# mmetcalf14/qml-cutensornet

Measured on AMD Instinct MI355X. Metric: Gram kernel entries/sec @ 60 qubits x 6 layers, higher is better.
Workload: dtype f64 (complex128)

## Files before the change

qml-cutensornet_amd/csrc/qk_fused.h:

```cpp
#pragma once
#include "qk_device.h"
#include "qk_plan.h"

#define QKF_PRIO_LO() __builtin_amdgcn_s_setprio(0)
#define QKF_PRIO_HI() __builtin_amdgcn_s_setprio(2)
typedef double v2d __attribute__((ext_vector_type(2)));
typedef __attribute__((address_space(3))) v2d lds_v2d;
static constexpr int QKF_XSTEP = 4 * TILE;
static constexpr int QKF_XBLOCK = TILE * TILE;


#ifndef QKF_LDS3M
#define QKF_LDS3M 0
#endif
#ifndef QKF_P2_PROBE
#define QKF_P2_PROBE 0
#endif
#ifndef QKF_ABL
#define QKF_ABL 0
#endif
#define QKF_STEP_BARRIER()                            \
  do {                                                \
    if (QKF_ABL & 4) asm volatile("s_waitcnt lgkmcnt(0)" ::: "memory"); \
    else qk_lds_barrier();                            \
// ... 219 lines not shown
  }
}

#ifdef QKF_EDGE_PAIRS_V
#define QKF_EDGE_PAIRS(WPS) (QKF_EDGE_PAIRS_V != 0)
#else
#define QKF_EDGE_PAIRS(WPS) false
#endif
#ifdef QKF_EDGE_SETS_V
#define QKF_EDGE_SETS(WPS) (QKF_EDGE_SETS_V)
#else
#define QKF_EDGE_SETS(WPS) ((WPS) <= 3 ? 2 : 1)
#endif
__device__ __forceinline__ v2d qkf_lde(const v2d* __restrict__ base, const unsigned boff, const int col = 0) {
  return reinterpret_cast<const v2d*>(reinterpret_cast<const char*>(base) + (size_t)boff)[col];
}
template <bool HAS1, bool MORE>
__device__ __forceinline__ void qkf_edge_group(v4d (&acc)[6], v2d (&fy)[4], v2d (&fz)[4], v2d (&fx)[4], const v2d* const* const by, const v2d* const* const bx, const unsigned boy,
                                               const unsigned box) {
#pragma unroll
  for (int i = 0; i < 4; ++i) {
    const double sb = QKF_DIF(fx[i].x, fx[i].y);
    acc[0] = __builtin_amdgcn_mfma_f64_16x16x4f64(fy[i].x, fx[i].x, acc[0], 0, 0, 0);
    acc[1] = __builtin_amdgcn_mfma_f64_16x16x4f64(fy[i].y, fx[i].y, acc[1], 0, 0, 0);
    acc[2] = __builtin_amdgcn_mfma_f64_16x16x4f64(QKF_SUM(fy[i].x, fy[i].y), sb, acc[2], 0, 0, 0);
    if (HAS1) {
      acc[3] = __builtin_amdgcn_mfma_f64_16x16x4f64(fz[i].x, fx[i].x, acc[3], 0, 0, 0);
      acc[4] = __builtin_amdgcn_mfma_f64_16x16x4f64(fz[i].y, fx[i].y, acc[4], 0, 0, 0);
      acc[5] = __builtin_amdgcn_mfma_f64_16x16x4f64(QKF_SUM(fz[i].x, fz[i].y), sb, acc[5], 0, 0, 0);
    }
    if (MORE) {
      fy[i] = qkf_lde(by[i], boy);
      if (HAS1) fz[i] = qkf_lde(by[i], boy, TILE);
      fx[i] = qkf_lde(bx[i], box);
    }
    __builtin_amdgcn_sched_barrier(0);
  }
}
template <bool HAS1, int SETS>
__device__ __forceinline__ void qkf_edge_unit(QkfTile& t0, QkfTile& t1, const v2d* __restrict__ Ay, const unsigned oy, const int ldy, const v2d* __restrict__ Ax, const unsigned ox, const int ldx,
                                              const int ng) {
  static_assert(SETS == 1 || SETS == 2, "one or two groups of k-steps in flight");
  v4d acc[6];
#pragma unroll
  for (int e = 0; e < 6; ++e) acc[e] = (v4d){0, 0, 0, 0};
  v2d fy[SETS][4], fz[SETS][4], fx[SETS][4];
  const v2d *by[4 * SETS], *bx[4 * SETS];
#pragma unroll
  for (int i = 0; i < 4 * SETS; ++i) by[i] = Ay + 4 * i * ldy, bx[i] = Ax + 4 * i * ldx;
  unsigned boy = oy * 16u, box = ox * 16u;
  const unsigned sy = (unsigned)(SETS * TILE * ldy) * 16u, sx = (unsigned)(SETS * TILE * ldx) * 16u;
  const bool two = SETS == 2 && ng > 1;
#pragma unroll
  for (int s = 0; s < SETS; ++s) {
    if (s == 0 || two) {
#pragma unroll
      for (int i = 0; i < 4; ++i) {
        fy[s][i] = qkf_lde(by[4 * s + i], boy);
        if (HAS1) fz[s][i] = qkf_lde(by[4 * s + i], boy, TILE);
        fx[s][i] = qkf_lde(bx[4 * s + i], box);
      }
    }
  }
  QKF_PRIO_LO();
#pragma unroll 1
  for (int g = SETS; g < ng; g += SETS) {
    boy += sy, box += sx;
#pragma unroll
    for (int s = 0; s < SETS; ++s) qkf_edge_group<HAS1, true>(acc, fy[s], fz[s], fx[s], by + 4 * s, bx + 4 * s, boy, box);
  }
  qkf_edge_group<HAS1, false>(acc, fy[0], fz[0], fx[0], by, bx, boy, box);
  if constexpr (SETS == 2) {
    if (two) qkf_edge_group<HAS1, false>(acc, fy[1], fz[1], fx[1], by + 4, bx + 4, boy, box);
  }
  QKF_PRIO_HI();
  t0.re = acc[0] + acc[1], t0.im = acc[2] - acc[0] + acc[1];
  if (HAS1) t1.re = acc[3] + acc[4], t1.im = acc[5] - acc[3] + acc[4];
}
__device__ __forceinline__ long long qkf_uniform(const long long v) {
  const unsigned lo = __builtin_amdgcn_readfirstlane((unsigned)v);
  const unsigned hi = __builtin_amdgcn_readfirstlane((unsigned)((unsigned long long)v >> 32));
  return (long long)(((unsigned long long)hi << 32) | lo);
}

template <int NW, bool PAIRS>
__device__ __forceinline__ QkEdgeUnit qkf_edge_unit_of(const int u, const int mt, const int nt, const int inv) {
  if constexpr (PAIRS) return qk_edge_unit(u, mt, nt, NW, inv);
  const int tb = (u * inv) >> 20;
  return QkEdgeUnit{u - tb * mt, tb, false, true};
}
template <int NW, bool PAIRS, int SETS>
__device__ __forceinline__ void qkf_edge_prefix(const SweepArgs& g, const int xi, const int yj, const int a, const int b, lds_v2d* const xl, v2d* const xg, const bool to_global, const int wave,
                                                const int q, const int j) {
  const v2d* const Lx = reinterpret_cast<const v2d*>(g.xedge) + qkf_uniform(g.xedge_offs[2 * (long long)xi]);
  const v2d* const Ly = reinterpret_cast<const v2d*>(g.yedge) + qkf_uniform(g.yedge_offs[2 * (long long)yj]);
  const int mt = a / TILE, nt = b / TILE, ng = (1 << g.edge_k) >> 4, inv = qk_recip20(mt), units = PAIRS ? qk_edge_units(mt, nt, NW) : mt * nt;
  for (int u = wave; u < units; u += NW) {
    const QkEdgeUnit un = qkf_edge_unit_of<NW, PAIRS>(u, mt, nt, inv);
    if (!un.mine) continue;
    QkfTile T0, T1;
    const unsigned oy = (unsigned)(q * b + un.tb0 * TILE + j), ox = (unsigned)(q * a + un.ta * TILE + j);
    if (un.has1) qkf_edge_unit<true, 1>(T0, T1, Ly, oy, b, Lx, ox, a, ng);
    else qkf_edge_unit<false, SETS>(T0, T1, Ly, oy, b, Lx, ox, a, ng);
    const int at = un.ta * (b * TILE) + (un.tb0 * TILE + q) * TILE + j;
    if (to_global) {
#pragma unroll
      for (int r = 0; r < 4; ++r) xg[at + r * QKF_XSTEP] = (v2d){T0.re[r], T0.im[r]};
      if (un.has1) {
#pragma unroll
        for (int r = 0; r < 4; ++r) xg[at + QKF_XBLOCK + r * QKF_XSTEP] = (v2d){T1.re[r], T1.im[r]};
      }
    } else {
#pragma unroll
      for (int r = 0; r < 4; ++r) xl[at + r * QKF_XSTEP] = (v2d){T0.re[r], T0.im[r]};
      if (un.has1) {
#pragma unroll
        for (int r = 0; r < 4; ++r) xl[at + QKF_XBLOCK + r * QKF_XSTEP] = (v2d){T1.re[r], T1.im[r]};
      }
    }
  }
}

template <int NW, bool PAIRS, int SETS>
__device__ __forceinline__ void qkf_edge_suffix(const SweepArgs& g, const int xi, const int yj, const int a, const int b, const lds_v2d* const xl, const v2d* const xg, const bool from_global,
                                                __attribute__((address_space(3))) double* zacc, const int wave, const int q, const int j) {
  const v2d* const Rx = reinterpret_cast<const v2d*>(g.xedge) + qkf_uniform(g.xedge_offs[2 * (long long)xi + 1]);
  const v2d* const Ry = reinterpret_cast<const v2d*>(g.yedge) + qkf_uniform(g.yedge_offs[2 * (long long)yj + 1]);
  const int mt = a / TILE, nt = b / TILE, ng = (1 << g.edge_k) >> 4, inv = qk_recip20(mt), units = PAIRS ? qk_edge_units(mt, nt, NW) : mt * nt;
  double zr = 0, zi = 0;
  for (int u = wave; u < units; u += NW) {
    const QkEdgeUnit un = qkf_edge_unit_of<NW, PAIRS>(u, mt, nt, inv);
    if (!un.mine) continue;
    QkfTile T0, T1;
    const unsigned oy = (unsigned)(q * b + un.tb0 * TILE + j), ox = (unsigned)(q * a + un.ta * TILE + j);
    if (un.has1) qkf_edge_unit<true, 1>(T0, T1, Ry, oy, b, Rx, ox, a, ng);
    else qkf_edge_unit<false, SETS>(T0, T1, Ry, oy, b, Rx, ox, a, ng);
    const int at = un.ta * (b * TILE) + (un.tb0 * TILE + q) * TILE + j;
#pragma unroll
    for (int r = 0; r < 4; ++r) {
      const v2d x = from_global ? xg[at + r * QKF_XSTEP] : (v2d)xl[at + r * QKF_XSTEP];
      zr += x.x * T0.re[r] - x.y * T0.im[r], zi += x.x * T0.im[r] + x.y * T0.re[r];
    }
    if (un.has1) {
#pragma unroll
      for (int r = 0; r < 4; ++r) {
        const v2d x = from_global ? xg[at + QKF_XBLOCK + r * QKF_XSTEP] : (v2d)xl[at + QKF_XBLOCK + r * QKF_XSTEP];
        zr += x.x * T1.re[r] - x.y * T1.im[r], zi += x.x * T1.im[r] + x.y * T1.re[r];
      }
    }
  }
#pragma unroll
  for (int o = 32; o > 0; o >>= 1) zr += __shfl_xor(zr, o), zi += __shfl_xor(zi, o);
  if ((q | j) == 0) zacc[2 * wave] = zr, zacc[2 * wave + 1] = zi;
}

struct QkfSite {
  int a, a2, b, b2, at, nks, mt, nt, nn, W, inv, inv2, pd, ps, next;
  bool small;
  const v2d *Ak, *Bk;
};
typedef int v4i __attribute__((ext_vector_type(4)));
typedef __attribute__((address_space(3))) v4i lds_v4i;

template <int XCAP, int NT, bool ITEM_RECIPS = false, typename OneRound>
__device__ __forceinline__ void qkf_step_table(const SweepArgs& g, const int xi, const int yj, lds_v4i* const rec, long long* const m_off, const int tid, const OneRound one_round) {
  const int ns = g.n_sites, n1 = ns + 1;
  const int32_t* const xd = g.xdims + (long long)xi * n1;
  const int32_t* const yd = g.ydims + (long long)yj * n1;
  const int32_t* const xt = g.xtrue + (long long)xi * n1;
  const int32_t* const yt = g.ytrue + (long long)yj * n1;
  const v2d* const xdata = reinterpret_cast<const v2d*>(g.xdata);
  const v2d* const ydata = reinterpret_cast<const v2d*>(g.ydata);
  auto is_small = [&](const int a, const int a2, const int b, const int b2, const int pd) __attribute__((always_inline)) {
    return a * b <= XCAP && a2 * b2 <= XCAP && (one_round(pd * (a / TILE), b2 / TILE) || a * b + a2 * b2 <= XCAP);
  };
  auto put = [&](const int e, const int a, const int a2, const int b, const int b2, const int ps, const int next, const bool small, const v2d* const A, const v2d* const B)
                 __attribute__((always_inline)) {
    const int mt = a / TILE, nt = b2 / TILE;
    const int W = small ? nt : max(1, min(nt, XCAP / (TILE * a2)));
    rec[3 * e] = (v4i){a, a2, b, b2};
    rec[3 * e + 1] = (v4i){xt[e], (yt[e] + 3) >> 2, W, small ? 1 : 0};
    rec[3 * e + 2] = (v4i){qk_recip20(mt), ps, next, ITEM_RECIPS ? qk_unit_recips(nt, W, false) : 0};
    m_off[2 * e] = (long long)(((const char*)A - (const char*)xdata) / 16);
    m_off[2 * e + 1] = (long long)(((const char*)B - (const char*)ydata) / 16);
  };
  auto plain = [&](const int e, const int next) __attribute__((always_inline)) {
    const int a = xd[e], a2 = xd[e + 1], b = yd[e], b2 = yd[e + 1];
    put(e, a, a2, b, b2, 1, next, is_small(a, a2, b, b2, 2), xdata + (g.xoffs[(long long)xi * ns + e] >> 1), ydata + (g.yoffs[(long long)yj * ns + e] >> 1));
  };
  if (g.merge_steps == 0) {
    for (int e = tid; e < ns; e += NT) plain(e, e + 1);
    return;
  }
  const int ek = g.edge_k, k_hi = ns - ek;
  for (int t = tid; 2 * t < k_hi - ek; t += NT) {
    const int e = ek + 2 * t;
    if (e + 1 >= k_hi) {
      plain(e, e + 1);
      continue;
    }
    const int a = xd[e], am = xd[e + 1], a2 = xd[e + 2], b = yd[e], bm = yd[e + 1], b2 = yd[e + 2];
    const bool sm = is_small(a, a2, b, b2, 4);
    const long long work_m = 4ll * a * b2 * (b + a2), work_p = 2ll * a * bm * (b + am) + 2ll * am * b2 * (bm + a2);
    const bool merged = (sm || (!is_small(a, am, b, bm, 2) && !is_small(am, a2, bm, b2, 2))) && work_m <= work_p;
    plain(e + 1, e + 2);
    if (merged)
      put(e, a, a2, b, b2, 2, e + 2, sm, reinterpret_cast<const v2d*>(g.xmg) + (g.xmg_offs[(long long)xi * g.merge_steps + t] >> 1),
          reinterpret_cast<const v2d*>(g.ymg) + (g.ymg_offs[(long long)yj * g.merge_steps + t] >> 1));
    else plain(e, e + 1);
  }
}

#ifdef QKF_PROF
#define QKF_PROF_DECL() \
  unsigned long long pf[8] = {0, 0, 0, 0, 0, 0, 0, 0}, pt = __builtin_amdgcn_s_memtime(); \
  const unsigned long long pt0 = pt
#define QKF_STAMP(i)                                              \
  do {                                                            \
    const unsigned long long now_ = __builtin_amdgcn_s_memtime(); \
    pf[i] += now_ - pt;                                           \
    pt = now_;                                                    \
  } while (0)
#define QKF_PROF_FLUSH()                                             \
  do {                                                               \
    if (lane == 0) {                                                 \
      pf[7] = __builtin_amdgcn_s_memtime() - pt0;                    \
      for (int i_ = 0; i_ < 8; ++i_) atomicAdd(g.prof + i_, pf[i_]); \
    }                                                                \
  } while (0)
#else
#define QKF_PROF_DECL()
#define QKF_STAMP(i)
#define QKF_PROF_FLUSH()
#endif

#define QKF_PULLER(NT) ((NT) - 64)
__device__ __forceinline__ void qkf_pull_next(const SweepArgs& g, const int xcc, int& gang_round, long long* const word) {
  const long long pp = qk_pull(g, xcc);
  qk_gang_sync(g, xcc, pp >= 0, gang_round);
  *word = pp;
}

template <int NW, int S, int XCAP, int WPS, bool DET = false>
__global__ __launch_bounds__(64 * NW, WPS) void qk_sweep_fused_kernel(const SweepArgs g) {
  constexpr int NT = 64 * NW;
  extern __shared__ __attribute__((aligned(16))) double lds_raw[];
  lds_v2d* const XL = (lds_v2d*)lds_raw;
  long long* const slot = reinterpret_cast<long long*>(lds_raw + 2 * XCAP);
  const v2d* const xdata = reinterpret_cast<const v2d*>(g.xdata);
  const v2d* const ydata = reinterpret_cast<const v2d*>(g.ydata);
  v2d* const G0 = reinterpret_cast<v2d*>(g.scratch) + (long long)blockIdx.x * 2 * g.x_plane;
  const int tid = threadIdx.x, lane = tid & 63;
  const int wave = __builtin_amdgcn_readfirstlane(tid >> 6);
  const int j = lane & 15, q = lane >> 4;
  const int ns = g.n_sites;
  __attribute__((address_space(3))) double* const zacc = (__attribute__((address_space(3))) double*)(slot + 2);
  lds_v4i* const rec = (lds_v4i*)(slot + 2 + 32);
  long long* const m_off = reinterpret_cast<long long*>(slot + 2 + 32) + 6 * (long long)ns;
  lds_int* const tbroken = (lds_int*)(m_off + 2 * (long long)ns);
  lds_int* const turn0 = tbroken + 2;
  auto rfl = [&](const int v) __attribute__((always_inline)) { return __builtin_amdgcn_readfirstlane(v); };
  auto ldl = [&](const long long* p_) __attribute__((always_inline)) {
    const long long v = *p_;
    const unsigned lo = __builtin_amdgcn_readfirstlane((unsigned)v);
    const unsigned hi = __builtin_amdgcn_readfirstlane((unsigned)((unsigned long long)v >> 32));
    return (long long)(((unsigned long long)hi << 32) | lo);
  };
  auto site = [&](const int k) __attribute__((always_inline)) {
    const v4i r0 = rec[3 * k], r1 = rec[3 * k + 1], r2 = rec[3 * k + 2];
    QkfSite s;
    s.a = rfl(r0.x), s.a2 = rfl(r0.y), s.b = rfl(r0.z), s.b2 = rfl(r0.w);
    s.at = rfl(r1.x), s.nks = rfl(r1.y), s.W = rfl(r1.z), s.small = rfl(r1.w) != 0;
    s.inv = rfl(r2.x), s.inv2 = rfl(r2.w);
    s.ps = rfl(r2.y), s.pd = 1 << s.ps, s.next = rfl(r2.z);
    s.mt = s.a / TILE, s.nt = s.b2 / TILE, s.nn = s.a2 / TILE;
    s.Ak = xdata + ldl(m_off + 2 * k);
    s.Bk = ydata + ldl(m_off + 2 * k + 1);
    return s;
  };
  auto item_of = [&](const QkfSite& s, const int w, const int it) __attribute__((always_inline)) {
    return DET ? qk_unit_decode_ordered(it, s.ps, s.mt, s.inv) : qk_unit_decode(it, s.mt, w, s.inv, qk_unit_recip_of(s.inv2, w == s.W));
  };
  auto b_stream = [&](const QkfSite& s, const int s0, const int w, const int it) __attribute__((always_inline)) {
    const QkUnit un = item_of(s, w, it);
    return QkfStream{s.Bk + un.p * s.b2, (unsigned)((q * s.pd) * s.b2 + (s0 + un.tc) * TILE + j), 4 * s.pd * s.b2, min(4, s.nks)};
  };
  auto a_stream = [&](const QkfSite& s, const int w, const int it) __attribute__((always_inline)) {
    const QkUnit un = item_of(s, w, it);
    return QkfStream{s.Ak + un.p * s.a2, (unsigned)(((un.ta * TILE + q) * s.pd) * s.a2 + j), 4 * s.pd * s.a2, min(4, (s.at - un.ta * TILE + 3) >> 2)};
  };
  QKF_PROF_DECL();
  const int xcc = qk_xcc_id();
  int gang_round = 0;
  if (tid == 0) qk_tail_start(g);
  for (;;) {
    if (tid == 0) {
      const long long pp_ = qk_pull(g, xcc);
      qk_gang_sync(g, xcc, pp_ >= 0, gang_round);
      *slot = pp_;
    }
    __syncthreads();
    const long long p = *slot;
    __syncthreads();
    if (p < 0) break;
    const int xi = g.pairs[2 * p], yj = g.pairs[2 * p + 1];
    qkf_step_table<XCAP, NT, true>(g, xi, yj, rec, m_off, tid, [](const int pmt, const int nt) { return pmt * nt <= NW * S; });
// ... 226 lines not shown
#endif
      p1 = __builtin_amdgcn_mfma_f64_16x16x4f64(s0[i], fr[i].x, p1, 0, 0, 0);
      p2 = __builtin_amdgcn_mfma_f64_16x16x4f64(t0.re[i], sp, p2, 0, 0, 0);
      p3 = __builtin_amdgcn_mfma_f64_16x16x4f64(t0.im[i], sm, p3, 0, 0, 0);
      if (HAS1) {
        r1 = __builtin_amdgcn_mfma_f64_16x16x4f64(s1[i], fr[i].x, r1, 0, 0, 0);
        r2 = __builtin_amdgcn_mfma_f64_16x16x4f64(t1.re[i], sp, r2, 0, 0, 0);
        r3 = __builtin_amdgcn_mfma_f64_16x16x4f64(t1.im[i], sm, r3, 0, 0, 0);
      }
    }
    if (!(QKF_ABL & 2)) fr[i] = qkf_ldg_a(i == 0 ? b0 : i == 1 ? b1 : i == 2 ? b2 : b3, off);
    __builtin_amdgcn_sched_barrier(0);
  }
  QKF_PRIO_HI();
#if QKF_LDS3M
#pragma unroll
  for (int r = 0; r < 4; ++r) {
    __hip_atomic_fetch_add(d + r * rs, p1[r], __ATOMIC_RELAXED, __HIP_MEMORY_SCOPE_WORKGROUP);
    __hip_atomic_fetch_add(d + r * rs + 1, p1[r], __ATOMIC_RELAXED, __HIP_MEMORY_SCOPE_WORKGROUP);
    __hip_atomic_fetch_add(d + r * rs, p3[r], __ATOMIC_RELAXED, __HIP_MEMORY_SCOPE_WORKGROUP);
    __hip_atomic_fetch_add(d + r * rs + 1, p2[r], __ATOMIC_RELAXED, __HIP_MEMORY_SCOPE_WORKGROUP);
  }
  if (HAS1) {
#pragma unroll
    for (int r = 0; r < 4; ++r) {
      __hip_atomic_fetch_add(d1 + r * rs, r1[r], __ATOMIC_RELAXED, __HIP_MEMORY_SCOPE_WORKGROUP);
      __hip_atomic_fetch_add(d1 + r * rs + 1, r1[r], __ATOMIC_RELAXED, __HIP_MEMORY_SCOPE_WORKGROUP);
      __hip_atomic_fetch_add(d1 + r * rs, r3[r], __ATOMIC_RELAXED, __HIP_MEMORY_SCOPE_WORKGROUP);
      __hip_atomic_fetch_add(d1 + r * rs + 1, r2[r], __ATOMIC_RELAXED, __HIP_MEMORY_SCOPE_WORKGROUP);
    }
  }
#elif QKF_P2_PROBE
  {
    const v4d re = p1 - p3, im = p1 - p2, re1 = r1 - r3, im1 = r1 - r2;
    lds_double* const e = d - (threadIdx.x & 63);
    lds_double* const e1 = e + 2 * QKF_XBLOCK;
#pragma unroll
    for (int r = 0; r < 4; ++r) {
      if (QKF_P2_PROBE == 1) {
        __hip_atomic_fetch_add(e + r * 64, re[r], __ATOMIC_RELAXED, __HIP_MEMORY_SCOPE_WORKGROUP);
        __hip_atomic_fetch_add(e + r * 64 + 256, im[r], __ATOMIC_RELAXED, __HIP_MEMORY_SCOPE_WORKGROUP);
        if (HAS1) {
          __hip_atomic_fetch_add(e1 + r * 64, re1[r], __ATOMIC_RELAXED, __HIP_MEMORY_SCOPE_WORKGROUP);
          __hip_atomic_fetch_add(e1 + r * 64 + 256, im1[r], __ATOMIC_RELAXED, __HIP_MEMORY_SCOPE_WORKGROUP);
        }
      } else if (QKF_P2_PROBE == 2) {
        *(lds_v2d*)(d + r * rs) = (v2d){re[r], im[r]};
        if (HAS1) *(lds_v2d*)(d1 + r * rs) = (v2d){re1[r], im1[r]};
      } else if (QKF_P2_PROBE == 3) {
        asm volatile("" ::"v"(re[r]), "v"(im[r]), "v"(re1[r]), "v"(im1[r]));
      } else {
        asm volatile("" ::"v"(p1[r]), "v"(p2[r]), "v"(p3[r]), "v"(r1[r]), "v"(r2[r]), "v"(r3[r]));
      }
    }
  }
#else
  {
    const v4d re = p1 - p3, im = p1 - p2;
#pragma unroll
    for (int r = 0; r < 4; ++r) {
      __hip_atomic_fetch_add(d + r * rs, re[r], __ATOMIC_RELAXED, __HIP_MEMORY_SCOPE_WORKGROUP);
      __hip_atomic_fetch_add(d + r * rs + 1, im[r], __ATOMIC_RELAXED, __HIP_MEMORY_SCOPE_WORKGROUP);
    }
  }
  if (HAS1) {
    const v4d re = r1 - r3, im = r1 - r2;
#pragma unroll
    for (int r = 0; r < 4; ++r) {
      __hip_atomic_fetch_add(d1 + r * rs, re[r], __ATOMIC_RELAXED, __HIP_MEMORY_SCOPE_WORKGROUP);
      __hip_atomic_fetch_add(d1 + r * rs + 1, im[r], __ATOMIC_RELAXED, __HIP_MEMORY_SCOPE_WORKGROUP);
    }
  }
#endif
}
template <bool FULL, bool HAS1, bool DET>
__device__ __forceinline__ void qkf_p2_dual_turn(const QkfTile& t0, const QkfTile& t1, v2d (&fr)[4], v2d (&fs)[4], QkfStream cur, const int ps, const int nn, const int kmax, lds_v2d* xo, const int q,
                                            const int j, const QkfStream nxt, const bool nxt_p1, const unsigned n1, const QkfTurn turn = QkfTurn{nullptr, 0, nullptr, nullptr}) {
  __attribute__((address_space(3))) double* d = (__attribute__((address_space(3))) double*)(xo + q * TILE + j);
#pragma unroll 1
  for (int tn = 0; tn < nn; ++tn) {
    v4d p1 = {0, 0, 0, 0}, p2 = {0, 0, 0, 0}, p3 = {0, 0, 0, 0}, r1 = {0, 0, 0, 0}, r2 = {0, 0, 0, 0}, r3 = {0, 0, 0, 0};
    const bool fin = tn + 1 == nn;
    const v2d* const rb = fin ? nxt.base : cur.base;
    const int rs = fin ? nxt.step : cur.step;
    cur.off = fin ? nxt.off : cur.off + TILE;
    QKF_PRIO_LO();
#pragma unroll
    for (int i = 0; i < 4; ++i) {
      if (FULL || i < kmax) {
        qkf_kstep<true>(p1, p2, p3, t0.re[i], t0.im[i], fr[i].x, fr[i].y);
        if (HAS1) qkf_kstep<true>(r1, r2, r3, t1.re[i], t1.im[i], fr[i].x, fr[i].y);
      }
      fr[i] = qkf_ldg_a(rb + i * rs, cur.off);
      __builtin_amdgcn_sched_barrier(0);
    }
    QKF_PRIO_HI();
    {
      const v4d re = p1 + p2, im = p3 - p1 + p2;
      if constexpr (DET) qkf_turn_add(d, (long)2 * QKF_XSTEP, re, im, turn, tn);
      else {
#pragma unroll
        for (int r = 0; r < 4; ++r) {
          __hip_atomic_fetch_add(d + r * 2 * QKF_XSTEP, re[r], __ATOMIC_RELAXED, __HIP_MEMORY_SCOPE_WORKGROUP);
          __hip_atomic_fetch_add(d + r * 2 * QKF_XSTEP + 1, im[r], __ATOMIC_RELAXED, __HIP_MEMORY_SCOPE_WORKGROUP);
        }
      }
    }
    if (HAS1) {
      const v4d re = r1 + r2, im = r3 - r1 + r2;
      __attribute__((address_space(3))) double* const d1 = d + 2 * QKF_XBLOCK;
      if constexpr (DET) qkf_turn_add(d1, (long)2 * QKF_XSTEP, re, im, QkfTurn{turn.at + nn, turn.idx, turn.broken, turn.gerr}, tn);
      else {
#pragma unroll
        for (int r = 0; r < 4; ++r) {
          __hip_atomic_fetch_add(d1 + r * 2 * QKF_XSTEP, re[r], __ATOMIC_RELAXED, __HIP_MEMORY_SCOPE_WORKGROUP);
          __hip_atomic_fetch_add(d1 + r * 2 * QKF_XSTEP + 1, im[r], __ATOMIC_RELAXED, __HIP_MEMORY_SCOPE_WORKGROUP);
        }
      }
    }
    d += 2 * ps;
  }
}

template <bool FULL, bool HAS1, bool DET = false>
__device__ __forceinline__ void qkf_p2_dual(const QkfTile& t0, const QkfTile& t1, v2d (&fr)[4], v2d (&fs)[4], QkfStream cur, const int ps, const int nn, const int kmax, lds_v2d* xo, const int q,
                                            const int j, const QkfStream nxt, const bool nxt_p1, const unsigned n1, const QkfTurn turn = QkfTurn{nullptr, 0, nullptr, nullptr}) {
  if constexpr (DET) {
    qkf_p2_dual_turn<FULL, HAS1, DET>(t0, t1, fr, fs, cur, ps, nn, kmax, xo, q, j, nxt, nxt_p1, n1, turn);
    return;
  }
  lds_double* d = (lds_double*)(xo + q * TILE + j);
  lds_double* d1 = d + 2 * QKF_XBLOCK;
  constexpr long rs = 2 * QKF_XSTEP;
  const v4d s0 = t0.re + t0.im, s1 = HAS1 ? t1.re + t1.im : s0;
  const v2d *const c0 = cur.base, *const c1 = cur.base + cur.step, *const c2 = cur.base + 2 * cur.step, *const c3 = cur.base + 3 * cur.step;
  unsigned off = cur.off;
#pragma unroll 1
  for (int tn = 0; tn + 1 < nn; ++tn) {
    off += TILE;
    qkf_p2_block<FULL, HAS1>(t0, t1, s0, s1, fr, kmax, c0, c1, c2, c3, off, d, d1, rs);
    d += 2 * ps, d1 += 2 * ps;
  }
  qkf_p2_block<FULL, HAS1>(t0, t1, s0, s1, fr, kmax, nxt.base, nxt.base + nxt.step, nxt.base + 2 * nxt.step, nxt.base + 3 * nxt.step, nxt.off, d, d1, rs);
}

template <int NW, int XCAP, int WPS, bool DET = false>
__global__ __launch_bounds__(64 * NW, WPS) void qk_sweep_fused_dual_kernel(const SweepArgs g) {
  constexpr int NT = 64 * NW;
  extern __shared__ __attribute__((aligned(16))) double lds_raw[];
  lds_v2d* const XL = (lds_v2d*)lds_raw;
  long long* const slot = reinterpret_cast<long long*>(lds_raw + 2 * XCAP);
  const v2d* const xdata = reinterpret_cast<const v2d*>(g.xdata);
  const v2d* const ydata = reinterpret_cast<const v2d*>(g.ydata);
  v2d* const G0 = reinterpret_cast<v2d*>(g.scratch) + (long long)blockIdx.x * 2 * g.x_plane;
  const int tid = threadIdx.x, lane = tid & 63;
  const int wave = __builtin_amdgcn_readfirstlane(tid >> 6);
  const int j = lane & 15, q = lane >> 4;
  const int ns = g.n_sites;
  __attribute__((address_space(3))) double* const zacc = (__attribute__((address_space(3))) double*)(slot + 2);
  lds_v4i* const rec = (lds_v4i*)(slot + 2 + 32);
  long long* const m_off = reinterpret_cast<long long*>(slot + 2 + 32) + 6 * (long long)ns;
  lds_int* const tbroken = (lds_int*)(m_off + 2 * (long long)ns);
  lds_int* const turn0 = tbroken + 2;
  auto rfl = [&](const int v) __attribute__((always_inline)) { return __builtin_amdgcn_readfirstlane(v); };
  auto ldl = [&](const long long* p_) __attribute__((always_inline)) {
    const long long v = *p_;
    const unsigned lo = __builtin_amdgcn_readfirstlane((unsigned)v);
    const unsigned hi = __builtin_amdgcn_readfirstlane((unsigned)((unsigned long long)v >> 32));
    return (long long)(((unsigned long long)hi << 32) | lo);
  };
  auto site = [&](const int k) __attribute__((always_inline)) {
    const v4i r0 = rec[3 * k], r1 = rec[3 * k + 1], r2 = rec[3 * k + 2];
    QkfSite s;
    s.a = rfl(r0.x), s.a2 = rfl(r0.y), s.b = rfl(r0.z), s.b2 = rfl(r0.w);
    s.at = rfl(r1.x), s.nks = rfl(r1.y), s.W = rfl(r1.z), s.small = rfl(r1.w) != 0;
    s.inv = rfl(r2.x);
    s.ps = rfl(r2.y), s.pd = 1 << s.ps, s.next = rfl(r2.z);
    s.mt = s.a / TILE, s.nt = s.b2 / TILE, s.nn = s.a2 / TILE;
    s.Ak = xdata + ldl(m_off + 2 * k);
    s.Bk = ydata + ldl(m_off + 2 * k + 1);
    return s;
  };
  auto pair_of = [&](const QkfSite& s, const int v) __attribute__((always_inline)) { return qk_unit_decode_ordered(v, s.ps, s.mt, s.inv); };
  auto b_stream = [&](const QkfSite& s, const int s0, const int v, const int half) __attribute__((always_inline)) {
    const QkUnit un = pair_of(s, v);
    return QkfStream{s.Bk + un.p * s.b2, (unsigned)((q * s.pd) * s.b2 + (s0 + 2 * un.tc + half) * TILE + j), 4 * s.pd * s.b2};
  };
  struct Unit {
    bool mine, has1;
    int v, half;
  };
  auto unit_of = [&](const QkfSite& s, const int w, const int units, const int r0) __attribute__((always_inline)) {
    Unit un;
    const int left = units - r0;
    const bool halves = 2 * left <= NW;
    un.half = (halves && wave >= left) ? 1 : 0;
    un.v = r0 + wave - (un.half ? left : 0);
    const int tp = pair_of(s, un.v).tc;
    const bool second = 2 * tp + 1 < w;
    un.mine = un.v < units && (un.half == 0 || second);
    un.has1 = !halves && second;
    return un;
  };
  auto a_stream = [&](const QkfSite& s, const int v) __attribute__((always_inline)) {
    const QkUnit un = pair_of(s, v);
    return QkfStream{s.Ak + un.p * s.a2, (unsigned)(((un.ta * TILE + q) * s.pd) * s.a2 + j), 4 * s.pd * s.a2};
  };
  QKF_PROF_DECL();
  const int xcc = qk_xcc_id();
  int gang_round = 0;
  if (tid == 0) qk_tail_start(g);
  if (tid == QKF_PULLER(NT)) qkf_pull_next(g, xcc, gang_round, slot);
  __syncthreads();
  long long p = slot[0];
  int psel = 0;
  auto table_of = [&](const long long pp) __attribute__((always_inline)) {
    if (pp < 0) return;
    const int xi_ = g.pairs[2 * pp], yj_ = g.pairs[2 * pp + 1];
    qkf_step_table<XCAP, NT>(g, xi_, yj_, rec, m_off, tid, [](const int pmt, const int nt) { return pmt * ((nt + 1) / 2) <= NW; });
  };
  table_of(p);
  while (p >= 0) {
    const int xi = g.pairs[2 * p], yj = g.pairs[2 * p + 1];
    const int ek = g.edge_k, k_hi = ns - ek;
    const bool edges = ek > 0;
    if (!edges)
      for (int e = tid; e < TILE * TILE; e += NT) XL[e] = (v2d){e == 0 ? 1.0 : 0.0, 0.0};
    if constexpr (DET)
      for (int e = tid; e < 2 * g.turn_ints + 2; e += NT) tbroken[e] = 0;
    int tsel = 0;
    __syncthreads();
    bool xg = false;
    int cur = 0, xb = 0;
    if (edges) {
      const v4i r0 = rec[3 * ek];
      const int a_e = rfl(r0.x), b_e = rfl(r0.z);
      xg = a_e * b_e > XCAP;
      qkf_edge_prefix<NW, QKF_EDGE_PAIRS(WPS), QKF_EDGE_SETS(WPS)>(g, xi, yj, a_e, b_e, XL, G0, xg, wave, q, j);
      __syncthreads();
    }
    QKF_STAMP(0);
    QkfTile T0, T1;
    v2d fr[4], fs[4];
    bool primed = false;
    QkfSite sn = site(ek);
    for (int k = ek; k < k_hi;) {
      const QkfSite sc = sn;
      k = sc.next;
      if (k < k_hi) sn = site(k);
      const int a = sc.a, a2 = sc.a2, b = sc.b, mt = sc.mt, nt = sc.nt, W = sc.W;
      const bool small = sc.small;
      v2d* const Gc = G0 + (long long)cur * g.x_plane;
      v2d* const Gn = G0 + (long long)(cur ^ 1) * g.x_plane;
      if (small && xg) {
        for (int e = tid; e < a * b; e += NT) XL[e] = Gc[e];
        __syncthreads();
        xg = false, xb = 0;
      } else if (!small && !xg) {
        for (int e = tid; e < a * b; e += NT) Gc[e] = XL[xb + e];
        __syncthreads();
        xg = true;
      }
      const int n_out = sc.b2 * a2;
      const bool pingpong = small && a * b + n_out <= XCAP;
      const int ob = !small ? 0 : pingpong ? (xb == 0 ? XCAP - n_out : 0) : 0;
      if (pingpong && !DET)
        for (int e = tid; e < n_out; e += NT) XL[ob + e] = (v2d){0.0, 0.0};
      QKF_STAMP(1);
      for (int s0 = 0; s0 < nt; s0 += W) {
        const int w = min(W, nt - s0), units = sc.pd * mt * ((w + 1) >> 1);
        lds_int* const tcur = turn0 + tsel * g.turn_ints;
        if constexpr (DET) {
          for (int e = tid; e < g.turn_ints; e += NT) turn0[(tsel ^ 1) * g.turn_ints + e] = 0;
        } else if (!small) {
          for (int e = tid; e < w * TILE * a2; e += NT) XL[e] = (v2d){0.0, 0.0};
          QKF_STEP_BARRIER();
        }
        for (int r0 = 0; r0 < units; r0 += NW) {
          const Unit un = unit_of(sc, w, units, r0);
          const int v = un.v;
          const bool mine = un.mine, has1 = un.has1;
          const QkUnit pr = pair_of(sc, v);
          const int tp = pr.tc, ta = pr.ta;
          if (mine) {
            const QkfStream bs = b_stream(sc, s0, v, un.half), as = a_stream(sc, v);
            const unsigned xoff = (unsigned)(ta * (b * TILE) + q * TILE + j);
            if (xg) {
              if (has1) qkf_p1_dual<true>(T0, T1, fr, fs, primed, bs, (const v2d*)Gc, xoff, sc.nks, as);
              else qkf_p1_dual<false>(T0, T1, fr, fs, primed, bs, (const v2d*)Gc, xoff, sc.nks, as);
            } else {
              if (has1) qkf_p1_dual<true>(T0, T1, fr, fs, primed, bs, (const lds_v2d*)(XL + xb), xoff, sc.nks, as);
              else qkf_p1_dual<false>(T0, T1, fr, fs, primed, bs, (const lds_v2d*)(XL + xb), xoff, sc.nks, as);
            }
          }
          QKF_STAMP(2);
          if (small && r0 == 0 && !(DET && pingpong)) {
            QKF_STEP_BARRIER();
            if (!pingpong && !DET) {
              for (int e = tid; e < n_out; e += NT) XL[e] = (v2d){0.0, 0.0};
              QKF_STEP_BARRIER();
            }
          }
          QKF_STAMP(3);
          if (mine) {
            const int kmax = min(4, (sc.at - ta * TILE + 3) >> 2);
            QkfStream nxt = a_stream(sc, v);
            bool np1 = false;
            if (r0 + NW < units) {
              const Unit nu = unit_of(sc, w, units, r0 + NW);
              if (nu.mine) nxt = b_stream(sc, s0, nu.v, nu.half), np1 = true;
            } else if (s0 + W < nt) {
              const int w2 = min(W, nt - s0 - W);
              const Unit nu = unit_of(sc, w2, sc.pd * mt * ((w2 + 1) >> 1), 0);
              if (nu.mine) nxt = b_stream(sc, s0 + W, nu.v, nu.half), np1 = true;
            } else if (k < k_hi) {
              const int w2 = min(sn.W, sn.nt);
              const Unit nu = unit_of(sn, w2, sn.pd * sn.mt * ((w2 + 1) >> 1), 0);
              if (nu.mine) nxt = b_stream(sn, 0, nu.v, nu.half), np1 = true;
            }
            const unsigned nd1 = 0;
            lds_v2d* const xo = XL + ob + (2 * tp + un.half) * QKF_XBLOCK;
            const QkfTurn tp_turn{tcur + (2 * tp + un.half) * sc.nn, sc.pd * ta + pr.p, tbroken, g.err};
            if (has1) {
              if (kmax == 4) qkf_p2_dual<true, true, DET>(T0, T1, fr, fs, a_stream(sc, v), w * QKF_XBLOCK, sc.nn, 4, xo, q, j, nxt, np1, nd1, tp_turn);
              else qkf_p2_dual<false, true, DET>(T0, T1, fr, fs, a_stream(sc, v), w * QKF_XBLOCK, sc.nn, kmax, xo, q, j, nxt, np1, nd1, tp_turn);
            } else {
              if (kmax == 4) qkf_p2_dual<true, false, DET>(T0, T1, fr, fs, a_stream(sc, v), w * QKF_XBLOCK, sc.nn, 4, xo, q, j, nxt, np1, nd1, tp_turn);
              else qkf_p2_dual<false, false, DET>(T0, T1, fr, fs, a_stream(sc, v), w * QKF_XBLOCK, sc.nn, kmax, xo, q, j, nxt, np1, nd1, tp_turn);
            }
            primed = np1;
          }
          QKF_STAMP(4);
        }
        QKF_STEP_BARRIER();
        tsel ^= 1;
        QKF_STAMP(5);
        if (!small && nt > W) {
          for (int tn = 0; tn < sc.nn; ++tn)
            for (int e = tid; e < w * QKF_XBLOCK; e += NT) Gn[(long long)tn * (sc.b2 * TILE) + s0 * QKF_XBLOCK + e] = XL[tn * w * QKF_XBLOCK + e];
          __syncthreads();
        }
      }
      if (!small) {
        if (nt > W) cur ^= 1;
        else xg = false, xb = 0;
      } else {
        xb = ob;
      }
    }
    if (tid == QKF_PULLER(NT)) qkf_pull_next(g, xcc, gang_round, slot + (psel ^ 1));
    if (edges) {
      const v4i r0 = rec[3 * (k_hi - 1)];
      const int a_e = rfl(r0.y), b_e = rfl(r0.w);
      qkf_edge_suffix<NW, QKF_EDGE_PAIRS(WPS), QKF_EDGE_SETS(WPS)>(g, xi, yj, a_e, b_e, (const lds_v2d*)(XL + xb), (const v2d*)(G0 + (long long)cur * g.x_plane), xg, zacc, wave, q, j);
    }
    __syncthreads();
    const long long pn = slot[psel ^ 1];
    if (tid == 0) {
      v2d zz = {0.0, 0.0};
      if (edges)
        for (int w_ = 0; w_ < NW; ++w_) zz.x += zacc[2 * w_], zz.y += zacc[2 * w_ + 1];
      else zz = xg ? G0[(long long)cur * g.x_plane] : (v2d)XL[xb];
      g.values[p] = zz.x * zz.x + zz.y * zz.y;
      if (g.z) {
        g.z[2 * p] = zz.x;
        g.z[2 * p + 1] = zz.y;
      }
    }
    table_of(pn);
    if (!edges) __syncthreads();
    p = pn, psel ^= 1;
    QKF_STAMP(6);
  }
  if (tid == 0) qk_tail_exit(g);
  QKF_PROF_FLUSH();
}

template <typename T>
__global__ void qk_interleave_kernel(const T* __restrict__ src, T* __restrict__ dst, const int32_t* __restrict__ dims, const int64_t* __restrict__ offs,
                                     const int n_sites, const long long n_tensors) {
  typedef T v2 __attribute__((ext_vector_type(2)));
  for (long long t = blockIdx.x; t < n_tensors; t += gridDim.x) {
    const long long s = t / n_sites;
    const int k = (int)(t - s * n_sites);
    const long long plane = (long long)dims[s * (n_sites + 1) + k] * 2 * dims[s * (n_sites + 1) + k + 1];
    const T* re = src + offs[t];
    const T* im = re + plane;
    v2* d = reinterpret_cast<v2*>(dst + offs[t]);
    for (long long e = threadIdx.x; e < plane; e += blockDim.x) d[e] = (v2){re[e], im[e]};
  }
}

template <int N>
__device__ __forceinline__ void qkw_wait_vmcnt() {
  static_assert(N >= 0 && N < 64, "vmcnt is a 6-bit field");
  asm volatile("s_waitcnt vmcnt(%0)" ::"n"(N) : "memory");
}

template <int NG, typename SRC>
__global__ __launch_bounds__(64, 2) void qk_sweep_wave2_kernel(const SweepArgs g) {
  constexpr bool F32 = sizeof(SRC) == 4;
  static_assert(!F32 || NG > 0, "complex64 images go through the LDS ring");
  constexpr int ES = F32 ? 8 : 16;
  constexpr int GROUP = F32 ? 128 : 256;
  __shared__ long long slot;
  __shared__ v2d ring[NG > 0 ? NG * GROUP : 1];
  typedef __attribute__((address_space(3))) void* lds_ptr_t;
  const int lane = threadIdx.x, j = lane & 15, q = lane >> 4;
  const unsigned ring_lds = (unsigned)(uintptr_t)(lds_ptr_t)ring + (F32 ? (unsigned)(q * 128 + j * 8) : (unsigned)lane * 16u);
  const int ns = g.n_sites, n1 = ns + 1;
  const char* const xdata = reinterpret_cast<const char*>(g.xdata);
  const char* const ydata = reinterpret_cast<const char*>(g.ydata);
  auto uni = [](const int v) __attribute__((always_inline)) { return __builtin_amdgcn_readfirstlane(v); };
  auto unil = [](const long long v) __attribute__((always_inline)) {
    const unsigned lo = __builtin_amdgcn_readfirstlane((unsigned)v);
    const unsigned hi = __builtin_amdgcn_readfirstlane((unsigned)((unsigned long long)v >> 32));
    return (long long)(((unsigned long long)hi << 32) | lo);
  };
  const int xcc = qk_xcc_id();
  if (lane == 0) qk_tail_start(g);
  for (;;) {
    if (lane == 0) slot = qk_pull(g, xcc);
    __syncthreads();
    const long long p = unil(slot);
    __syncthreads();
    if (p < 0) break;
    typedef const __attribute__((address_space(4))) int* sint_p;
    typedef const __attribute__((address_space(4))) int64_t* slong_p;
    const int xi = ((sint_p)g.pairs)[2 * p], yj = ((sint_p)g.pairs)[2 * p + 1];
    const sint_p xd = (sint_p)(g.xdims + (long long)xi * n1);
    const sint_p yd = (sint_p)(g.ydims + (long long)yj * n1);
    const sint_p xt = (sint_p)(g.xtrue + (long long)xi * n1);
    const sint_p yt = (sint_p)(g.ytrue + (long long)yj * n1);
    const slong_p xo = (slong_p)(g.xoffs + (long long)xi * ns);
    const slong_p yo = (slong_p)(g.yoffs + (long long)yj * ns);
    QkfTile XA[2][2], XN[2][2];
#pragma unroll
    for (int u = 0; u < 2; ++u)
#pragma unroll
      for (int v = 0; v < 2; ++v) XA[u][v].re = XA[u][v].im = XN[u][v].re = XN[u][v].im = (v4d){0, 0, 0, 0};
    XA[0][0].re[0] = (lane == 0) ? 1.0 : 0.0;
    int f_k = 0, f_i = 0, f_n = 0, f_slot = 0, c_slot = 0;
    int f_a2 = 0, f_b2 = 0;
    const char* f_A = xdata;
    const char* f_B = ydata;
    int desc = 0;
    auto enter = [&]() __attribute__((always_inline)) {
      const int fa = xd[f_k], fb = yd[f_k], fat = __builtin_amdgcn_readfirstlane(xt[f_k]), fbt = __builtin_amdgcn_readfirstlane(yt[f_k]);
      f_a2 = xd[f_k + 1], f_b2 = yd[f_k + 1];
      f_A = xdata + (xo[f_k] >> 1) * ES, f_B = ydata + (yo[f_k] >> 1) * ES;
      const int kb = fb >> 4, nn = f_a2 >> 4, mt = fa >> 4, nt = f_b2 >> 4, gpb = kb + nn;
      const int inv = (gpb == 2) ? 32768 : (gpb == 3) ? 21846 : 16384;
      const int gi = lane, blk = (gi * inv) >> 16, h = gi - blk * gpb, pp = blk & 1, r = blk >> 1;
      const int ta = (mt == 2) ? (r & 1) : 0, tb = (mt == 2) ? (r >> 1) : r;
      const bool is_b = h < kb;
      const int off = is_b ? ((h * TILE) * 2 + pp) * f_b2 + tb * TILE : ((ta * TILE) * 2 + pp) * f_a2 + (h - kb) * TILE;
      const int cnt = is_b ? min(4, (fbt - h * TILE + 3) >> 2) : min(4, (fat - ta * TILE + 3) >> 2);
      desc = off | (cnt << 16) | ((is_b ? 1 : 0) << 20);
      f_n = nt * mt * 2 * gpb, f_i = 0;
    };
    auto issue = [&]() __attribute__((always_inline)) {
      if (f_k >= ns) return;
      const int d = __builtin_amdgcn_readlane(desc, f_i);
      const int off = d & 0xffff, cnt = (d >> 16) & 7;
      const bool is_b = (d >> 20) != 0;
      const int ld = is_b ? f_b2 : f_a2;
      const char* const base = (is_b ? f_B : f_A) + (long)off * ES;
      if constexpr (F32) {
        const char* const src = base + (((lane >> 3) * 2) * ld + (lane & 7) * 2) * ES;
        const int last = (cnt - 1) >> 1;
#pragma unroll
        for (int pc = 0; pc < 2; ++pc) if (!(QKF_ABL & 16)) __builtin_amdgcn_global_load_lds(src + (min(pc, last) * 16 * ld) * ES, (lds_ptr_t)(ring + f_slot * GROUP + pc * 64), 16, 0, 0);
      } else {
        const char* const src = base + ((q * 2) * ld + j) * ES;
#pragma unroll
        for (int i = 0; i < 4; ++i) if (!(QKF_ABL & 16)) __builtin_amdgcn_global_load_lds(src + (min(i, cnt - 1) * 8 * ld) * ES, (lds_ptr_t)(ring + (f_slot * 4 + i) * 64), 16, 0, 0);
      }
      f_slot = (f_slot == NG - 1) ? 0 : f_slot + 1;
      if (++f_i == f_n) {
        if (++f_k < ns) enter();
      }
    };
    auto take = [&](v2d(&f)[4]) __attribute__((always_inline)) {
      issue();
      if (f_k >= ns) qkw_wait_vmcnt<0>();
      else qkw_wait_vmcnt<(NG > 0 ? (F32 ? 2 : 4) * (NG - 1) : 0)>();
      const unsigned at = ring_lds + (unsigned)c_slot * (unsigned)(GROUP * 16);
      if constexpr (F32) {
        double h[4];
        asm volatile("ds_read_b64 %0, %1" : "=v"(h[0]) : "v"(at));
        asm volatile("ds_read_b64 %0, %1 offset:512" : "=v"(h[1]) : "v"(at));
        asm volatile("ds_read_b64 %0, %1 offset:1024" : "=v"(h[2]) : "v"(at));
// ... 107 lines not shown
```

Before: 698,700.

## Carry next-unit decode across rounds and unroll LDS zero/copy loops

Restructures the fused sweep loop so the unit decode and B-stream for the next round are computed once and carried forward, instead of being recomputed both for prefetch and for the current round. Site metadata is split into a lookahead part and a per-step part, and asm constraints pin round values in scalar registers. LDS zero and copy loops become 4-way unrolled helpers. The aim is to cut scalar/vector integer overhead and improve memory-level parallelism in the staging copies, at the cost of more live registers and more complex state carried between rounds.

```diff
diff --git a/qml-cutensornet_amd/csrc/qk_fused.h b/qml-cutensornet_amd/csrc/qk_fused.h
--- a/qml-cutensornet_amd/csrc/qk_fused.h
+++ b/qml-cutensornet_amd/csrc/qk_fused.h
@@ -395,6 +395,36 @@
 #pragma unroll
   for (int o = 32; o > 0; o >>= 1) zr += __shfl_xor(zr, o), zi += __shfl_xor(zi, o);
   if ((q | j) == 0) zacc[2 * wave] = zr, zacc[2 * wave + 1] = zi;
+}
+
+template <int NT>
+__device__ __forceinline__ void qkf_zero(lds_v2d* const base, const int n, const int tid) {
+  lds_v2d* at = base + tid;
+  int e = 0;
+#pragma unroll 1
+  for (; e + 4 * NT <= n; e += 4 * NT, at += 4 * NT) {
+#pragma unroll
+    for (int i = 0; i < 4; ++i) at[i * NT] = (v2d){0.0, 0.0};
+  }
+#pragma unroll 1
+  for (; e < n; e += NT, at += NT)
+    if (e + tid < n) *at = (v2d){0.0, 0.0};
+}
+template <int NT, typename Dst, typename Src>
+__device__ __forceinline__ void qkf_copy(Dst* const dst, const Src* const src, const int n, const int tid) {
+  int e = 0;
+  unsigned at = (unsigned)tid;
+#pragma unroll 1
+  for (; e + 4 * NT <= n; e += 4 * NT, at += 4 * NT) {
+    v2d v[4];
+#pragma unroll
+    for (int i = 0; i < 4; ++i) v[i] = src[at + i * NT];
+#pragma unroll
+    for (int i = 0; i < 4; ++i) dst[at + i * NT] = v[i];
+  }
+#pragma unroll 1
+  for (; e < n; e += NT, at += NT)
+    if (at < (unsigned)n) dst[at] = src[at];
 }
 
 struct QkfSite {
@@ -927,7 +957,7 @@
   long long* const slot = reinterpret_cast<long long*>(lds_raw + 2 * XCAP);
   const v2d* const xdata = reinterpret_cast<const v2d*>(g.xdata);
   const v2d* const ydata = reinterpret_cast<const v2d*>(g.ydata);
-  v2d* const G0 = reinterpret_cast<v2d*>(g.scratch) + (long long)blockIdx.x * 2 * g.x_plane;
+  v2d* const G0 = reinterpret_cast<v2d*>(g.scratch) + qkf_uniform((long long)blockIdx.x * 2 * g.x_plane);
   const int tid = threadIdx.x, lane = tid & 63;
   const int wave = __builtin_amdgcn_readfirstlane(tid >> 6);
   const int j = lane & 15, q = lane >> 4;
@@ -944,42 +974,54 @@
     const unsigned hi = __builtin_amdgcn_readfirstlane((unsigned)((unsigned long long)v >> 32));
     return (long long)(((unsigned long long)hi << 32) | lo);
   };
-  auto site = [&](const int k) __attribute__((always_inline)) {
+  struct Ahead {
+    int a, b2, W, inv, ps;
+    long long Bo;
+  };
+  auto ahead_of = [&](const int k) __attribute__((always_inline)) {
     const v4i r0 = rec[3 * k], r1 = rec[3 * k + 1], r2 = rec[3 * k + 2];
-    QkfSite s;
-    s.a = rfl(r0.x), s.a2 = rfl(r0.y), s.b = rfl(r0.z), s.b2 = rfl(r0.w);
-    s.at = rfl(r1.x), s.nks = rfl(r1.y), s.W = rfl(r1.z), s.small = rfl(r1.w) != 0;
-    s.inv = rfl(r2.x);
-    s.ps = rfl(r2.y), s.pd = 1 << s.ps, s.next = rfl(r2.z);
-    s.mt = s.a / TILE, s.nt = s.b2 / TILE, s.nn = s.a2 / TILE;
-    s.Ak = xdata + ldl(m_off + 2 * k);
-    s.Bk = ydata + ldl(m_off + 2 * k + 1);
-    return s;
-  };
-  auto pair_of = [&](const QkfSite& s, const int v) __attribute__((always_inline)) { return qk_unit_decode_ordered(v, s.ps, s.mt, s.inv); };
-  auto b_stream = [&](const QkfSite& s, const int s0, const int v, const int half) __attribute__((always_inline)) {
-    const QkUnit un = pair_of(s, v);
-    return QkfStream{s.Bk + un.p * s.b2, (unsigned)((q * s.pd) * s.b2 + (s0 + 2 * un.tc + half) * TILE + j), 4 * s.pd * s.b2};
+    return Ahead{rfl(r0.x), rfl(r0.w), rfl(r1.z), rfl(r2.x), rfl(r2.y), ldl(m_off + 2 * k + 1)};
+  };
+  struct Step {
+    int a, a2, b, b2, at, nks, W, inv, ps, next;
+    bool small;
+    long long Ao, Bo;
+  };
+  auto step_of = [&](const int k, const Ahead& h) __attribute__((always_inline)) {
+    const v4i r0 = rec[3 * k], r1 = rec[3 * k + 1], r2 = rec[3 * k + 2];
+    return Step{h.a, rfl(r0.y), rfl(r0.z), h.b2, rfl(r1.x), rfl(r1.y), h.W, h.inv, h.ps, rfl(r2.z), rfl(r1.w) != 0, ldl(m_off + 2 * k), h.Bo};
   };
   struct Unit {
     bool mine, has1;
-    int v, half;
-  };
-  auto unit_of = [&](const QkfSite& s, const int w, const int units, const int r0) __attribute__((always_inline)) {
+    int v, half, ta, tp, p;
+  };
+  auto unit_of = [&](const int ps, const int mt, const int inv, const int w, const int units, const int r0) __attribute__((always_inline)) {
     Unit un;
     const int left = units - r0;
     const bool halves = 2 * left <= NW;
     un.half = (halves && wave >= left) ? 1 : 0;
     un.v = r0 + wave - (un.half ? left : 0);
-    const int tp = pair_of(s, un.v).tc;
-    const bool second = 2 * tp + 1 < w;
+    const QkUnit pr = qk_unit_decode_ordered(un.v, ps, mt, inv);
+    un.ta = pr.ta, un.tp = pr.tc, un.p = pr.p;
+    const bool second = 2 * un.tp + 1 < w;
     un.mine = un.v < units && (un.half == 0 || second);
     un.has1 = !halves && second;
     return un;
   };
-  auto a_stream = [&](const QkfSite& s, const int v) __attribute__((always_inline)) {
-    const QkUnit un = pair_of(s, v);
-    return QkfStream{s.Ak + un.p * s.a2, (unsigned)(((un.ta * TILE + q) * s.pd) * s.a2 + j), 4 * s.pd * s.a2};
+  auto b_stream = [&](const long long Bo, const int b2, const int ps, const int s0, const Unit& un) __attribute__((always_inline)) {
+    return QkfStream{ydata + Bo + (un.p * b2 + (s0 + 2 * un.tp + un.half) * TILE), __umul24((unsigned)q, (unsigned)(b2 << ps)) + (unsigned)j, (4 * b2) << ps};
+  };
+  auto a_stream = [&](const Step& s, const Unit& un) __attribute__((always_inline)) {
+    return QkfStream{xdata + s.Ao + (un.p + ((un.ta * TILE) << s.ps)) * s.a2, __umul24((unsigned)q, (unsigned)(s.a2 << s.ps)) + (unsigned)j, (4 * s.a2) << s.ps};
+  };
+  struct Round {
+    int nks, at, w, units, ob, s0;
+  };
+  auto round_values = [&](const int nks, const int at, const int w, const int units, const int ob, const int s0) __attribute__((always_inline)) {
+    Round r{nks, at, w, units, ob, s0};
+    asm volatile("" : "+s"(r.nks), "+s"(r.at));
+    asm volatile("" : "+s"(r.w), "+s"(r.units), "+s"(r.ob), "+s"(r.s0));
+    return r;
   };
   QKF_PROF_DECL();
   const int xcc = qk_xcc_id();
@@ -1018,101 +1060,108 @@
     QkfTile T0, T1;
     v2d fr[4], fs[4];
     bool primed = false;
-    QkfSite sn = site(ek);
+    Ahead hn = ahead_of(ek);
+    Unit un;
+    QkfStream bs;
+    {
+      const int mt = hn.a >> 4, w = min(hn.W, hn.b2 >> 4);
+      un = unit_of(hn.ps, mt, hn.inv, w, (mt << hn.ps) * ((w + 1) >> 1), 0);
+      bs = b_stream(hn.Bo, hn.b2, hn.ps, 0, un);
+    }
     for (int k = ek; k < k_hi;) {
-      const QkfSite sc = sn;
+      const Step sc = step_of(k, hn);
       k = sc.next;
-      if (k < k_hi) sn = site(k);
-      const int a = sc.a, a2 = sc.a2, b = sc.b, mt = sc.mt, nt = sc.nt, W = sc.W;
+      const int a = sc.a, a2 = sc.a2, b = sc.b, mt = a >> 4, nt = sc.b2 >> 4, nn = a2 >> 4, W = sc.W;
       const bool small = sc.small;
       v2d* const Gc = G0 + (long long)cur * g.x_plane;
       v2d* const Gn = G0 + (long long)(cur ^ 1) * g.x_plane;
       if (small && xg) {
-        for (int e = tid; e < a * b; e += NT) XL[e] = Gc[e];
+        qkf_copy<NT>(XL, (const v2d*)Gc, a * b, tid);
         __syncthreads();
         xg = false, xb = 0;
       } else if (!small && !xg) {
-        for (int e = tid; e < a * b; e += NT) Gc[e] = XL[xb + e];
+        qkf_copy<NT>(Gc, (const lds_v2d*)(XL + xb), a * b, tid);
         __syncthreads();
         xg = true;
       }
       const int n_out = sc.b2 * a2;
       const bool pingpong = small && a * b + n_out <= XCAP;
       const int ob = !small ? 0 : pingpong ? (xb == 0 ? XCAP - n_out : 0) : 0;
-      if (pingpong && !DET)
-        for (int e = tid; e < n_out; e += NT) XL[ob + e] = (v2d){0.0, 0.0};
+      if (pingpong && !DET) qkf_zero<NT>(XL + ob, n_out, tid);
       QKF_STAMP(1);
       for (int s0 = 0; s0 < nt; s0 += W) {
-        const int w = min(W, nt - s0), units = sc.pd * mt * ((w + 1) >> 1);
+        const int w = min(W, nt - s0), units = (mt << sc.ps) * ((w + 1) >> 1);
         lds_int* const tcur = turn0 + tsel * g.turn_ints;
         if constexpr (DET) {
           for (int e = tid; e < g.turn_ints; e += NT) turn0[(tsel ^ 1) * g.turn_ints + e] = 0;
         } else if (!small) {
-          for (int e = tid; e < w * TILE * a2; e += NT) XL[e] = (v2d){0.0, 0.0};
+          qkf_zero<NT>(XL, w * TILE * a2, tid);
           QKF_STEP_BARRIER();
         }
         for (int r0 = 0; r0 < units; r0 += NW) {
-          const Unit un = unit_of(sc, w, units, r0);
-          const int v = un.v;
           const bool mine = un.mine, has1 = un.has1;
-          const QkUnit pr = pair_of(sc, v);
-          const int tp = pr.tc, ta = pr.ta;
+          const Round rv = round_values(sc.nks, sc.at, w, units, ob, s0);
+          const QkfStream as = a_stream(sc, un);
           if (mine) {
-            const QkfStream bs = b_stream(sc, s0, v, un.half), as = a_stream(sc, v);
-            const unsigned xoff = (unsigned)(ta * (b * TILE) + q * TILE + j);
+            const int xu = un.ta * (sc.b * TILE);
             if (xg) {
-              if (has1) qkf_p1_dual<true>(T0, T1, fr, fs, primed, bs, (const v2d*)Gc, xoff, sc.nks, as);
-              else qkf_p1_dual<false>(T0, T1, fr, fs, primed, bs, (const v2d*)Gc, xoff, sc.nks, as);
+              if (has1) qkf_p1_dual<true>(T0, T1, fr, fs, primed, bs, (const v2d*)Gc, (unsigned)(xu + q * TILE + j), rv.nks, as);
+              else qkf_p1_dual<false>(T0, T1, fr, fs, primed, bs, (const v2d*)Gc, (unsigned)(xu + q * TILE + j), rv.nks, as);
             } else {
-              if (has1) qkf_p1_dual<true>(T0, T1, fr, fs, primed, bs, (const lds_v2d*)(XL + xb), xoff, sc.nks, as);
-              else qkf_p1_dual<false>(T0, T1, fr, fs, primed, bs, (const lds_v2d*)(XL + xb), xoff, sc.nks, as);
+              if (has1) qkf_p1_dual<true>(T0, T1, fr, fs, primed, bs, (const lds_v2d*)(XL + xb), (unsigned)(xu + q * TILE + j), rv.nks, as);
+              else qkf_p1_dual<false>(T0, T1, fr, fs, primed, bs, (const lds_v2d*)(XL + xb), (unsigned)(xu + q * TILE + j), rv.nks, as);
             }
           }
           QKF_STAMP(2);
           if (small && r0 == 0 && !(DET && pingpong)) {
             QKF_STEP_BARRIER();
             if (!pingpong && !DET) {
-              for (int e = tid; e < n_out; e += NT) XL[e] = (v2d){0.0, 0.0};
+              qkf_zero<NT>(XL, n_out, tid);
               QKF_STEP_BARRIER();
             }
           }
           QKF_STAMP(3);
+          int n_ps = sc.ps, n_mt = mt, n_inv = sc.inv, n_b2 = sc.b2, n_s0 = rv.s0, n_w = rv.w, n_units = rv.units, n_r0 = r0 + NW;
+          long long n_Bo = sc.Bo;
+          bool any = true;
+          if (n_r0 < rv.units) {
+          } else if (rv.s0 + W < nt) {
+            n_s0 = rv.s0 + W, n_w = min(W, nt - n_s0), n_units = (mt << sc.ps) * ((n_w + 1) >> 1), n_r0 = 0;
+          } else if (k < k_hi) {
+            hn = ahead_of(k);
+            n_ps = hn.ps, n_mt = hn.a >> 4, n_inv = hn.inv, n_b2 = hn.b2, n_Bo = hn.Bo;
+            n_s0 = 0, n_w = min(hn.W, hn.b2 >> 4), n_units = (n_mt << n_ps) * ((n_w + 1) >> 1), n_r0 = 0;
+          } else {
+            any = false;
+          }
+          Unit nu = unit_of(n_ps, n_mt, n_inv, n_w, n_units, n_r0);
+          nu.mine = nu.mine && any;
+          const QkfStream nbs = b_stream(n_Bo, n_b2, n_ps, n_s0, nu);
           if (mine) {
-            const int kmax = min(4, (sc.at - ta * TILE + 3) >> 2);
-            QkfStream nxt = a_stream(sc, v);
-            bool np1 = false;
-            if (r0 + NW < units) {
-              const Unit nu = unit_of(sc, w, units, r0 + NW);
-              if (nu.mine) nxt = b_stream(sc, s0, nu.v, nu.half), np1 = true;
-            } else if (s0 + W < nt) {
-              const int w2 = min(W, nt - s0 - W);
-              const Unit nu = unit_of(sc, w2, sc.pd * mt * ((w2 + 1) >> 1), 0);
-              if (nu.mine) nxt = b_stream(sc, s0 + W, nu.v, nu.half), np1 = true;
-            } else if (k < k_hi) {
-              const int w2 = min(sn.W, sn.nt);
-              const Unit nu = unit_of(sn, w2, sn.pd * sn.mt * ((w2 + 1) >> 1), 0);
-              if (nu.mine) nxt = b_stream(sn, 0, nu.v, nu.half), np1 = true;
+            const int kmax = min(4, (rv.at - un.ta * TILE + 3) >> 2);
+            const QkfStream nxt = nu.mine ? nbs : as;
+            const bool np1 = nu.mine;
+            const unsigned nd1 = 0;
+            lds_v2d* const xo = XL + rv.ob + (2 * un.tp + un.half) * QKF_XBLOCK;
+            const QkfTurn tp_turn{tcur + (2 * un.tp + un.half) * (sc.a2 >> 4), (un.ta << sc.ps) + un.p, tbroken, g.err};
+            if (has1) {
+              if (kmax == 4) qkf_p2_dual<true, true, DET>(T0, T1, fr, fs, as, rv.w * QKF_XBLOCK, sc.a2 >> 4, 4, xo, q, j, nxt, np1, nd1, tp_turn);
+              else qkf_p2_dual<false, true, DET>(T0, T1, fr, fs, as, rv.w * QKF_XBLOCK, sc.a2 >> 4, kmax, xo, q, j, nxt, np1, nd1, tp_turn);
+            } else {
+              if (kmax == 4) qkf_p2_dual<true, false, DET>(T0, T1, fr, fs, as, rv.w * QKF_XBLOCK, sc.a2 >> 4, 4, xo, q, j, nxt, np1, nd1, tp_turn);
+              else qkf_p2_dual<false, false, DET>(T0, T1, fr, fs, as, rv.w * QKF_XBLOCK, sc.a2 >> 4, kmax, xo, q, j, nxt, np1, nd1, tp_turn);
             }
-            const unsigned nd1 = 0;
-            lds_v2d* const xo = XL + ob + (2 * tp + un.half) * QKF_XBLOCK;
-            const QkfTurn tp_turn{tcur + (2 * tp + un.half) * sc.nn, sc.pd * ta + pr.p, tbroken, g.err};
-            if (has1) {
-              if (kmax == 4) qkf_p2_dual<true, true, DET>(T0, T1, fr, fs, a_stream(sc, v), w * QKF_XBLOCK, sc.nn, 4, xo, q, j, nxt, np1, nd1, tp_turn);
-              else qkf_p2_dual<false, true, DET>(T0, T1, fr, fs, a_stream(sc, v), w * QKF_XBLOCK, sc.nn, kmax, xo, q, j, nxt, np1, nd1, tp_turn);
-            } else {
-              if (kmax == 4) qkf_p2_dual<true, false, DET>(T0, T1, fr, fs, a_stream(sc, v), w * QKF_XBLOCK, sc.nn, 4, xo, q, j, nxt, np1, nd1, tp_turn);
-              else qkf_p2_dual<false, false, DET>(T0, T1, fr, fs, a_stream(sc, v), w * QKF_XBLOCK, sc.nn, kmax, xo, q, j, nxt, np1, nd1, tp_turn);
-            }
-            primed = np1;
           }
+          primed = mine && nu.mine;
+          un = nu, bs = nbs;
           QKF_STAMP(4);
         }
         QKF_STEP_BARRIER();
         tsel ^= 1;
         QKF_STAMP(5);
         if (!small && nt > W) {
-          for (int tn = 0; tn < sc.nn; ++tn)
-            for (int e = tid; e < w * QKF_XBLOCK; e += NT) Gn[(long long)tn * (sc.b2 * TILE) + s0 * QKF_XBLOCK + e] = XL[tn * w * QKF_XBLOCK + e];
+          for (int tn = 0; tn < nn; ++tn)
+            qkf_copy<NT>(Gn + ((long long)tn * (sc.b2 * TILE) + s0 * QKF_XBLOCK), (const lds_v2d*)(XL + tn * w * QKF_XBLOCK), w * QKF_XBLOCK, tid);
           __syncthreads();
         }
       }
```

Measured after the change: 704,200, median of 6. No clear change (+0.8%).
